# LivGen/LMAT

Hardware: AMD Instinct MI355X
Metric: reads/s (150 bp) vs 64 GB k-mer DB (higher is better)
Workload: dtype u64; 1 GPU; 1104000000 x 150 bp reads/GPU vs 64 GiB k-mer hash (6467472668 20-mers, replicated per GPU), run_rl.sh flags -x 0 -j 30 -l 0 -b 1, calls-only; total_reads=1104000000, reads_per_launch=8000000, read_len=150, db_kmers=6467472668, k=20, parallelism=reads sharded x1, DB replicated, genus_block_permille=100, prune_g=0, list_replicas=1, distinct_lists=792576, reads_called=1058323347, read_pool_batches=32

## Files before the change

### lmat_amd/csrc/kernels.hip

```cpp
#include <hip/hip_runtime.h>
#include <atomic>
#include <type_traits>
#include "kernels.hpp"

#ifndef LMAT_ABLATE
#define LMAT_ABLATE 0
#endif
#define STOP_AT(n, v) do { if (LMAT_ABLATE && A.prm.stop_after == (n)) { if (lane == 0) { emit(250, (v)); } return; } } while (0)
#ifndef LMAT_CLOSURE_FAST
#define LMAT_CLOSURE_FAST 1
#endif
#ifndef LMAT_LDS_SHIFT
#define LMAT_LDS_SHIFT 0
#endif

namespace lmat {

#define WSYNC()                                              \
    do {                                                     \
        __builtin_amdgcn_fence(__ATOMIC_SEQ_CST, "wavefront"); \
        __builtin_amdgcn_wave_barrier();                     \
    } while (0)

template <bool GMEM>
// ... 1011 lines not shown
    float log_avg, stdev1;
    const float sc = k4_wave_stats(lane, nT, cand, my_cnt, xch, log_avg, stdev1);
    const float diff_thresh = stdev1 * Ap->prm.sdiff;
    const float s0 = __uint_as_float(rl(__float_as_uint(sc), (int)sx0));
    const float d = s0 - sc;
    uint64_t close = bal(d <= diff_thresh) & OTH;
    uint8_t match = LMAT_MT_DIRECT;
    uint32_t call_tid = rl(my_id, (int)sx0);
    float call_score = s0;
    if (close) {
        uint64_t good = CH;
        do {
            const uint32_t ivj = rl(fz.z, __builtin_ctzll(close));
            close &= close - 1;
            good &= bal(ti < (ivj & 0xFFFFu)) & bal((ivj >> 16) <= oi);
        } while (close && good);
        if (!good) {
            match = LMAT_MT_LCA_ERROR; call_tid = 0; call_score = 0;
        } else {
            const uint32_t k = wave_max_u32(lane_bit(good) ? (ti << 6) | (uint32_t)lane : 0u);
            match = LMAT_MT_MULTI; call_tid = rl(my_id, (int)(k & 63u));
        }
    }
    k4_wave_closed_record(Ap, lane, out, match, call_tid, call_score, cand, log_avg, stdev1, valid_kmers, len, bin_sel);
    return true;
}
#if LMAT_ABLATE
__device__ uint32_t g_path_why[16];
#define PATH_WHY(i) do { if (lane == 0) atomicAdd(&g_path_why[i], 1u); } while (0)
#else
#define PATH_WHY(i) ((void)0)
#endif
__device__ __forceinline__ bool k4_wave_path(CArgsK4* Ap, int lane, uint32_t nT, uint32_t cand, const u32x4 fz, uint32_t my_cnt,
                                             uint32_t my_id, uint32_t dep, uint32_t fl, uint32_t chain, uint32_t* xch, GAS uint64_t* out,
                                             int valid_kmers, uint32_t len, int bin_sel) {
    const uint32_t nK = (chain >> 8) & 0x7Fu;
    PATH_WHY(0);
    if (nK - 1u >= nT) { PATH_WHY(2); return false; }
    const uint64_t am = below_mask_1_64((int)nT);
    const uint32_t kv = wave_max_u32((uint32_t)lane < nK ? (my_cnt << 6) | (uint32_t)lane : 0u);
    const uint32_t v = kv & 63u, c0 = kv >> 6;
    const uint32_t ti = fz.z & 0xFFFFu, oi = fz.z >> 16;
    const uint32_t riv = rl(fz.z, (int)v);
    const uint32_t rt = riv & 0xFFFFu, ro = riv >> 16;
    const uint64_t CH = bal(ti < rt) & bal(ro <= oi) & am, PATH = CH | (1ull << v), OTH = am & ~PATH;
    if (!CH) { PATH_WHY(3); return false; }
    if (~bal(my_cnt < c0) & OTH) { PATH_WHY(4); return false; }
    if (~bal(my_cnt >= c0) & CH) { PATH_WHY(5); return false; }
    if (~(bal(oi < rt) | bal(ro < ti)) & OTH) { PATH_WHY(6); return false; }
    if (!(bal(dep == 0u) & CH)) { PATH_WHY(7); return false; }
    const uint32_t badfl = (uint32_t)kFlagPlasmid | (Ap->prm.screen_phix ? (uint32_t)kFlagPhiX : 0u);
    if (bal((fl & badfl) != 0)) { PATH_WHY(8); return false; }
    float log_avg, stdev1;
    const float sc = k4_wave_stats(lane, nT, cand, my_cnt, xch, log_avg, stdev1);
    const float diff_thresh = stdev1 * Ap->prm.sdiff;
    const float s0 = __uint_as_float(rl(__float_as_uint(sc), (int)v));
    uint64_t close = bal(s0 - sc <= diff_thresh) & OTH;
    uint8_t match = LMAT_MT_DIRECT;
    uint32_t call_tid = rl(my_id, (int)v);
    float call_score = s0;
    if (close) {
        uint64_t good = CH;
        do {
            const int j = __builtin_ctzll(close);
            close &= close - 1;
            const uint32_t ivj = rl(fz.z, j);
            const float sj = __uint_as_float(rl(__float_as_uint(sc), j));
            const uint64_t anc = bal(ti < (ivj & 0xFFFFu)) & bal((ivj >> 16) <= oi);
            if (bal(sc - sj > diff_thresh) & PATH & ~anc) { PATH_WHY(9); return false; }
            good &= anc;
        } while (close);
        if (!good) {
            match = LMAT_MT_LCA_ERROR; call_tid = 0; call_score = 0;
        } else {
            const uint32_t k = wave_max_u32(lane_bit(good) ? (ti << 6) | (uint32_t)lane : 0u);
            match = LMAT_MT_MULTI; call_tid = rl(my_id, (int)(k & 63u));
            call_score = __uint_as_float(wave_max_u32(lane_bit(PATH) && ti >= (k >> 6) ? __float_as_uint(sc) : 0u));
        }
    }
    PATH_WHY(1);
    k4_wave_closed_record(Ap, lane, out, match, call_tid, call_score, cand, log_avg, stdev1, valid_kmers, len, bin_sel);
    return true;
}
template <int THM, bool PLAIN = false>
__device__ __forceinline__ bool k4_wave(CArgsK4* Ap, int lane, uint32_t nT, uint32_t cand, const u32x4 fz, uint32_t my_cnt,
                                        uint32_t my_id, const unsigned int* hent, uint32_t* xch, GAS uint64_t* out,
                                        int valid_kmers, uint32_t len, int bin_sel, uint32_t chain = 0, uint32_t* took_chain = nullptr) {
    const float hbias = PLAIN ? 0.0f : Ap->prm.hbias, sdiff = Ap->prm.sdiff;
    const int screen_phix = Ap->prm.screen_phix;
    if (!PLAIN && !(Ap->prm.k4_static & 1)) return false;
    const int stop = LMAT_ABLATE ? Ap->prm.stop_after : 0;
    auto placeholder = [&]() {
        if (lane == 0) {
            uint32_t z = 0;
            asm volatile("" : "+v"(z));
            out[0] = (uint64_t)(z + ((uint32_t)LMAT_ST_SILENT | ((uint32_t)LMAT_MT_NOMATCH << 8) | (cand << 16))) | ((uint64_t)(uint32_t)valid_kmers << 32);
            out[1] = (uint64_t)len | ((uint64_t)z << 32);
            out[2] = (uint64_t)z | ((uint64_t)z << 32);
            out[3] = (uint64_t)z | ((uint64_t)z << 32);
            out[4] = (uint64_t)z | ((uint64_t)(uint32_t)bin_sel << 32);
        }
        return true;
    };
    if (stop == 30 || (stop == 34 && nT <= 16)) return placeholder();
    if (cand - 1u > 998u || nT - 1u > 63u) return false;
    const bool act = (uint32_t)lane < nT;
    const uint32_t dep = act ? (fz.w & 0xFFFFu) : 0u, fl = act ? (fz.w >> 16) : 0u;
    if (bal(my_cnt > cand) | bal(dep > 0x7FFFu) | (hbias != 0.0f ? bal((fl & kFlagHuman) != 0) : 0ull)) return false;
    if (LMAT_ABLATE && lane == 0) { G_ADD((GAS uint32_t*)Ap->cursor + kCurChainSeen, 1u); if (chain & 0x10000u) G_ADD((GAS uint32_t*)Ap->cursor + kCurChainLone, 1u); }
    if ((chain & 0x10000u) && (PLAIN || (Ap->prm.k4_static & 4)) &&
        k4_wave_chain(Ap, lane, nT, cand, fz, my_cnt, my_id, dep, fl, chain, xch, out, valid_kmers, len, bin_sel)) {
        if (LMAT_ABLATE && lane == 0) G_ADD((GAS uint32_t*)Ap->cursor + kCurChainTaken, 1u);
        if (took_chain) *took_chain = 1u;
        return true;
    }
    if ((chain & 0x20000u) && (PLAIN || (Ap->prm.k4_static & 8))) {
        if (LMAT_ABLATE && lane == 0) G_ADD((GAS uint32_t*)Ap->cursor + kCurPathSeen, 1u);
        if (k4_wave_path(Ap, lane, nT, cand, fz, my_cnt, my_id, dep, fl, chain, xch, out, valid_kmers, len, bin_sel)) {
            if (LMAT_ABLATE && lane == 0) G_ADD((GAS uint32_t*)Ap->cursor + kCurPathTaken, 1u);
            if (took_chain) *took_chain = 2u;
            return true;
        }
    }
    float* xs = (float*)xch;
    uint32_t* xk = xch + 64;
    uint32_t* xx = xch + 128;
    float* xv = (float*)(xch + 256);
    uint32_t* xp = xch + 320;
    const float fcand = (float)cand;
    const float sc = div_small_ints((float)my_cnt, fcand);
    xs[lane] = sc;
    uint32_t e = act ? (((my_cnt << 15) | dep) << 6) | (uint32_t)lane : 0xFFFFFFFFu;
    if (nT > 16) {
        int lg = 0;
        for (uint32_t t = nT; t > 1; t >>= 1) ++lg;
        uint32_t st0 = 0, st1 = 0, st2 = 0;
        int sp = 0, first = 0, last = (int)nT, depth = 2 * lg;
        bool busy = true;
        while (busy) {
            if (last - first <= 16) {
                if (sp > 0) {
                    --sp;
                    const uint32_t top = sp == 0 ? st0 : (sp == 1 ? st1 : st2);
                    first = (int)(top & 0xFFu); last = (int)((top >> 8) & 0xFFu); depth = (int)(top >> 16);
                } else busy = false;
            } else if (depth == 0) {
                return false;
            } else {
                --depth;
                const int ia = first + 1, ib = first + (last - first) / 2, ic = last - 1;
                const uint32_t ka = rl(e, ia) >> 6, kb = rl(e, ib) >> 6, kc = rl(e, ic) >> 6;
                const bool ab = ka < kb, bc = kb < kc, ac = ka < kc;
                const int pick = ab ? (bc ? ib : (ac ? ic : ia)) : (ac ? ia : (bc ? ic : ib));
                const uint32_t e_first = rl(e, first), e_pick = rl(e, pick);
                e = lane == first ? e_pick : (lane == pick ? e_first : e);
                const uint32_t K = e_pick >> 6;
                const uint64_t inr = below_mask(last) & ~below_mask(first + 1);
                const uint64_t GE = bal((e >> 6) >= K) & inr, LE = bal((e >> 6) <= K) & inr;
                const uint32_t pg = prefix_count(GE), pl = prefix_count(LE);
                const bool le = lane_bit(LE);
                const uint32_t above_le = (uint32_t)popc64(LE) - pl - (le ? 1u : 0u);
                const uint64_t SL = bal(above_le > pg) & GE;
                const uint64_t SR = bal(pg > above_le) & LE;
                int cut;
                if (SL) {
                    const bool swl = lane_bit(SL), swr = lane_bit(SR);
                    if (swl) xx[pg] = e;
                    if (swr) xx[64 + above_le] = e;
                    WSYNC();
                    if (swl) e = xx[64 + pg];
                    if (swr) e = xx[above_le];
                    WSYNC();
                    const int Lm = 63 - __builtin_clzll(SL), Rm = __builtin_ctzll(SR);
                    const uint64_t c = GE & ~below_mask(Lm + 1) & below_mask(Rm);
                    cut = c ? __builtin_ctzll(c) : Rm;
                } else {
                    cut = GE ? __builtin_ctzll(GE) : last;
                }
                if (last - cut > 16) {
                    const uint32_t v = (uint32_t)cut | ((uint32_t)last << 8) | ((uint32_t)depth << 16);
                    if (sp == 0) st0 = v; else if (sp == 1) st1 = v; else st2 = v;
                    ++sp;
                }
                last = cut;
            }
        }
    }
    const uint32_t keyr = act ? ((e & ~63u) | (uint32_t)lane) : 0xFFFFFFFFu;
    xk[lane] = keyr;
    WSYNC();
    float log_sum = 0.0f;
    uint32_t rank = 0;
    for (uint32_t t = 0; t < nT; t += 4) {
        const u32x4 q = *(const u32x4*)((const uint32_t*)xs + t);
        log_sum += __uint_as_float(q.x); log_sum += __uint_as_float(q.y); log_sum += __uint_as_float(q.z); log_sum += __uint_as_float(q.w);
        const u32x4 kq = *(const u32x4*)(xk + t);
        rank += (kq.x < keyr ? 1u : 0u) + (kq.y < keyr ? 1u : 0u) + (kq.z < keyr ? 1u : 0u) + (kq.w < keyr ? 1u : 0u);
    }
    const uint32_t pos_sig_hits = (uint32_t)popc64(bal(my_cnt > 0));
    const uint32_t use_sig_hits = pos_sig_hits > 3 ? pos_sig_hits : nT;
    const float log_avg = div_small_ints(log_sum, (float)use_sig_hits);
    const float dv = log_avg - sc;
    xv[lane] = act && (pos_sig_hits > 3 ? my_cnt > 0 : true) ? dv * dv : 0.0f;
// ... 1676 lines not shown
#pragma unroll
        for (int ch = 0; ch < EC; ++ch) {
            sreg[ch] = 0;
            if ((uint32_t)ch * 64 < nel) {
                const uint32_t e = (uint32_t)ch * 64 + lane;
                if (e < nel) {
                    const uint32_t sl = hent[tid_find(hent, THM, el_ta[e])] >> 16;
                    const bool el = !(dfl[el_d[e]] & kListNegFirst) && ((ES >> sl) & 1ull);
                    sreg[ch] = sl | (el ? 0x100u : 0u);
                    el_ta[e] = (uint16_t)sreg[ch];
                    if (el) atomicMin(&first[sl], e);
                }
            }
        }
        WSYNC();
        STOP_AT(43, nT);
        const uint64_t todo0 = __ballot(first[lane] != 0xFFFFFFFFu);
        const bool one = LMAT_CLOSURE_FAST && todo0 != 0 && (todo0 & (todo0 - 1)) == 0;
        const int sx0 = one ? __builtin_ctzll(todo0) : 0;
        if (one) {
            W = (uint32_t)__builtin_amdgcn_readlane((int)f_plen, sx0);
        } else {
#pragma unroll
            for (int ch = 0; ch < EC; ++ch) {
                if ((uint32_t)ch * 64 < nel) {
                    const uint32_t e = (uint32_t)ch * 64 + lane;
                    const uint32_t sl = sreg[ch] & 0xFFu;
                    const uint32_t plen = lane_of(f_plen, sl);
                    const bool walk = e < nel && first[sl] == e;
                    const uint32_t w = walk ? plen : 0u;
                    const uint32_t incl = wave_scan_incl(w);
                    if (e < nel) el_off[e] = (uint16_t)(W + incl - w);
                    W += (uint32_t)__builtin_amdgcn_readlane((int)incl, 63);
                }
            }
            WSYNC();
        }
        STOP_AT(44, W);
        if (W > 65535u) overflow = true;
        for (uint32_t i0 = 0; i0 < W && !overflow; i0 += 64) {
            const uint32_t i = i0 + lane;
            const bool act = i < W;
            uint32_t a = 0, h = 0;
            uint64_t pe = 0;
            uint32_t sl_i = 0, rel = 0;
            if (one) {
                sl_i = (uint32_t)sx0;
                rel = i;
            } else if (act) {
                uint32_t lo = 0, hi = nel;
                while (lo < hi) {
                    const uint32_t mid = (lo + hi) >> 1;
                    if ((uint32_t)el_off[mid] <= i) lo = mid + 1; else hi = mid;
                }
                const uint32_t e = lo - 1;
                sl_i = (uint32_t)el_ta[e] & 0xFFu;
                rel = i - (uint32_t)el_off[e];
            }
            const uint32_t poff_i = lane_of(f_poff, sl_i);
            uint32_t pf = 0;
            if (act) {
                pe = g_paths8[poff_i + rel];
                pf = ((const GAS uint8_t*)tb.paths_fl)[poff_i + rel];
                a = (uint32_t)(pe & 0xFFFFu);
                h = tid_find_or_claim(hent, THM, a);
                atomicMin(&hent[h], a | ((0x8000u | (uint32_t)lane) << 16));
            }
            WSYNC();
            const uint64_t nm_ = __ballot(i < W) & __ballot((hent[h] >> 16) == (0x8000u | (uint32_t)lane));
            const uint32_t newcnt = popc64(nm_);
            if (nT + newcnt > (uint32_t)T) { overflow = true; break; }
            if (lane_bit(nm_)) {
                const uint32_t s = nT + prefix_count(nm_);
                hent[h] = a | (s << 16);
                reg[s] = (uint16_t)a;
                anc_zw[s] = u32x2{(uint32_t)(pe >> 32), ((uint32_t)(pe >> 16) & 0xFFFFu) | (pf << 16)};
            }
            nT += newcnt;
            WSYNC();
        }
        STOP_AT(45, nT);
        if (!overflow && (uint32_t)lane >= nT_p1 && (uint32_t)lane < nT) { const u32x2 zw = anc_zw[lane]; fz = u32x4{0u, 0u, zw.x, zw.y}; }
        const bool lone = one && !overflow && W > 0 && nT - nT_p1 == W && cand == nuniq;
        if (!overflow) chain = 0x20000u | (nT_p1 << 8);
        if (lone) {
            const uint32_t c0 = cnt[sx0];
            if ((uint32_t)lane >= nT_p1 && (uint32_t)lane < nT) cnt[lane] = (uint16_t)c0;
            chain |= 0x10000u | (uint32_t)sx0;
            WSYNC();
        } else if (!overflow && W > 0) {
            const bool sl_act = (uint32_t)lane < nT;
            uint32_t tin_s = 0xFFFF, tout_s = 0;
            if (sl_act) { tin_s = fz.z & 0xFFFFu; tout_s = fz.z >> 16; }
            uint32_t anc_lo = 0, anc_hi = 0;
            uint64_t todo = todo0;
            while (todo) {
                const int sx = __builtin_ctzll(todo);
                todo &= todo - 1;
                const uint32_t tin_x = (uint32_t)__builtin_amdgcn_readlane((int)tin_s, sx);
                const uint32_t tout_x = (uint32_t)__builtin_amdgcn_readlane((int)tout_s, sx);
                const uint64_t am = __ballot(tin_s < tin_x) & __ballot(tout_x <= tout_s);
                uint32_t m0_keep;
                asm("s_mov_b32 %2, m0\n\ts_mov_b32 m0, %4\n\tv_writelane_b32 %0, %3, m0\n\tv_writelane_b32 %1, %5, m0\n\ts_mov_b32 m0, %2"
                    : "+v"(anc_lo), "+v"(anc_hi), "=&s"(m0_keep) : "s"((uint32_t)am), "s"(sx), "s"((uint32_t)(am >> 32)));
            }
            unsigned int* memw = (unsigned int*)el_t;
            unsigned int* hitw = (unsigned int*)el_off;
            static_assert(2 * E >= 512 && sizeof(*el_t) == 2 && sizeof(*el_off) == 2, "64 mask pairs fit each of the two dead arrays");
            *(u32x2*)(memw + 2 * lane) = u32x2{0u, 0u};
            *(u32x2*)(hitw + 2 * lane) = u32x2{0u, 0u};
            const bool wide_t = nT > 32u;
            WSYNC();
#pragma unroll
            for (int ch = 0; ch < EC; ++ch) {
                if ((uint32_t)ch * 64 < nel) {
                    const uint32_t e = (uint32_t)ch * 64 + lane;
                    const uint32_t se = e < nel ? (uint32_t)el_ta[e] : 0u;
                    const uint32_t sl = se & 0xFFu;
                    const uint32_t alo = lane_of(anc_lo, sl), ahi = wide_t ? lane_of(anc_hi, sl) : 0u;
                    if (e < nel) {
                        const uint32_t d2 = 2u * (uint32_t)el_d[e];
                        __hip_atomic_fetch_or(&memw[d2 + (sl >> 5)], 1u << (sl & 31u), __ATOMIC_RELAXED, __HIP_MEMORY_SCOPE_WORKGROUP);
                        if (se & 0x100u) {
                            __hip_atomic_fetch_or(&hitw[d2], alo, __ATOMIC_RELAXED, __HIP_MEMORY_SCOPE_WORKGROUP);
                            if (wide_t) __hip_atomic_fetch_or(&hitw[d2 + 1], ahi, __ATOMIC_RELAXED, __HIP_MEMORY_SCOPE_WORKGROUP);
                        }
                    }
                }
            }
            WSYNC();
            {
                const u32x2 me = *(const u32x2*)(memw + 2 * lane), hi_ = *(const u32x2*)(hitw + 2 * lane);
                *(u32x2*)(hitw + 2 * lane) = u32x2{hi_.x & ~me.x, hi_.y & ~me.y};
            }
            WSYNC();
            const unsigned int* aw = hitw + (lane >> 5);
            const uint32_t sh = (uint32_t)lane & 31u;
            uint32_t add = 0;
            auto mad_lo = [](uint32_t bit, uint32_t mm, uint32_t acc) -> uint32_t { uint32_t r; asm("v_mad_u32_u16 %0, %1, %2, %3" : "=v"(r) : "v"(bit), "v"(mm), "v"(acc)); return r; };
            auto mad_hi = [](uint32_t bit, uint32_t mm, uint32_t acc) -> uint32_t { uint32_t r; asm("v_mad_u32_u16 %0, %1, %2, %3 op_sel:[0,1,0,0]" : "=v"(r) : "v"(bit), "v"(mm), "v"(acc)); return r; };
            static_assert(L::D == 64 && (L::OFF_R2 + 4 * L::D) % 8 == 0, "the multiplicities are read eight bytes at a time, up to set 63");
            for (uint32_t d = 0; d < ndist; d += 4) {
                const unsigned int* pw = aw + 2 * d;
                const uint32_t w0 = pw[0], w1 = pw[2], w2 = pw[4], w3 = pw[6];
                const u32x2 mm = *(const u32x2*)(dmult + d);
                add = mad_lo(__builtin_amdgcn_ubfe(w0, sh, 1u), mm.x, add);
                add = mad_hi(__builtin_amdgcn_ubfe(w1, sh, 1u), mm.x, add);
                add = mad_lo(__builtin_amdgcn_ubfe(w2, sh, 1u), mm.y, add);
                add = mad_hi(__builtin_amdgcn_ubfe(w3, sh, 1u), mm.y, add);
            }
            if (sl_act && add) cnt[lane] = (uint16_t)(cnt[lane] + add);
            WSYNC();
        }
    }
    if (overflow) {
        if (lane == 0) {
            emit(255, 0);
            if (A.ovf_list) ((GAS uint32_t*)A.ovf_list)[G_ADD(&g_cursor[A.ovf_slot], 1u)] = (uint32_t)r;
            else G_OR(g_err, (uint32_t)kErrTidOverflow);
        }
        return;
    }
    STOP_AT(6, nT);
    if (!PLAIN && A.rand_max) {
        const uint32_t gcb = ((const GAS uint8_t*)A.rand_gc)[r - A.result_base];
        GAS uint32_t* rmax = (GAS uint32_t*)A.rand_max;
        GAS uint32_t* rcnt = (GAS uint32_t*)A.rand_cnt;
// ... 664 lines not shown
    if (!n) return;
    probe_stats_kernel<<<dim3((unsigned)((n + 255) / 256)), dim3(256), 0, stream>>>(tb, kmers, n, out);
}

void launch_gather_bench(const uint64_t* slots, uint32_t nbuckets, uint64_t n_probes, uint64_t seed,
                         unsigned long long* sink, hipStream_t stream, int bytes_per_probe) {
    const int grid = 256 * 16;
    if (bytes_per_probe == 128) {
        const uint64_t per_wave = (n_probes / grid + 71) / 72 * 72;
        gather_bench_kernel<8><<<dim3(grid), dim3(64), 0, stream>>>(slots, nbuckets, per_wave, seed, sink);
    } else {
        const uint64_t per_wave = (n_probes / grid + 143) / 144 * 144;
        gather_bench_kernel<4><<<dim3(grid), dim3(64), 0, stream>>>(slots, nbuckets, per_wave, seed, sink);
    }
}

template <int TT>
static void launch_k4_lds(const ClassifyArgs& a, uint64_t max_reads, hipStream_t stream) {
    using K = K4Lds<TT>;
    static PerDeviceOnce attr_once;
    attr_once([] { hipFuncSetAttribute((const void*)k4_lds_kernel<TT>, hipFuncAttributeMaxDynamicSharedMemorySize, K::BYTES); });
    const uint64_t per_cu = 160 * 1024 / K::BYTES;
    uint64_t g = (max_reads + K::LANES - 1) / K::LANES;
    if (g > 256 * per_cu) g = 256 * per_cu;
    static const int gcap = getenv("LMAT_K4_SMALL_GRID") ? atoi(getenv("LMAT_K4_SMALL_GRID")) : 0;
    if (TT == kK4SmallT && gcap > 0 && g > (uint64_t)gcap) g = gcap;
    if (g < 1) g = 1;
    k4_lds_kernel<TT><<<dim3((unsigned)g), dim3(64), K::BYTES, stream>>>(a);
}
void launch_k4_begin(const ClassifyArgs& a, hipStream_t stream, hipStream_t stream2, hipStream_t stream3, hipStream_t small_stream,
                     hipEvent_t forked) {
    uint64_t blocks = (a.count + 4095) / 4096;
    if (blocks > 256 * 8) blocks = 256 * 8;
    if (blocks < 1) blocks = 1;
    k4_compact_kernel<<<dim3((unsigned)blocks), dim3(256), 0, stream>>>(a);
    hipEventRecord(forked, stream);
    hipStreamWaitEvent(stream2, forked, 0);
    ClassifyArgs b = a;
    b.k4_slot = kCurK4Large;
    const uint64_t waves = (a.count + 63) / 64;
    uint64_t g2 = waves < 256 * 32 ? waves : 256 * 32;
    if (g2 < 1) g2 = 1;
    static const int g2cap = getenv("LMAT_K4_MID_GRID") ? atoi(getenv("LMAT_K4_MID_GRID")) : 0;
    if (g2cap > 0 && g2 > (uint64_t)g2cap) g2 = g2cap;
    else if (small_stream == stream3 && g2 > 1024) g2 = 1024;
    static const int mode = getenv("LMAT_K4_MODE") ? atoi(getenv("LMAT_K4_MODE")) : 0;
    if (a.nm.active) {
        k4_kernel<true, kK4T, 64><<<dim3((unsigned)g2), dim3(64), 0, stream2>>>(b);
    } else if (mode == 1) {
        launch_k4_lds<kK4MidT>(a, a.count, stream2);
    } else {
        b.k4_slot = kCurK4Mid;
        k4_kernel<false, kK4MidT, 64><<<dim3((unsigned)g2), dim3(64), 0, stream2>>>(b);
    }
    hipStreamWaitEvent(stream3, forked, 0);
    if (!a.nm.active && a.prm.k4_row) {
        uint64_t gr = (a.count + 3) / 4;
        if (gr > 256 * 64) gr = 256 * 64;
        if (gr < 1) gr = 1;
        k4_row_kernel<<<dim3((unsigned)gr), dim3(64), 0, stream3>>>(a);
    }
    if (!a.nm.active) launch_k4_lds<kK4T>(a, a.count / 8 + 64, stream3);
    if (small_stream != stream && small_stream != stream3) hipStreamWaitEvent(small_stream, forked, 0);
    launch_k4_lds<kK4SmallT>(a, a.count, small_stream);
}
void launch_k4_end(const ClassifyArgs& a, hipStream_t join_stream, hipStream_t stream2, hipStream_t stream3, hipStream_t small_stream,
                   hipEvent_t joined2, hipEvent_t joined3, hipEvent_t joined_small, hipEvent_t done) {
    if (stream2 != join_stream) { hipEventRecord(joined2, stream2); hipStreamWaitEvent(join_stream, joined2, 0); }
    if (stream3 != join_stream) { hipEventRecord(joined3, stream3); hipStreamWaitEvent(join_stream, joined3, 0); }
    if (small_stream != join_stream && small_stream != stream3 && small_stream != stream2) {
        hipEventRecord(joined_small, small_stream);
        hipStreamWaitEvent(join_stream, joined_small, 0);
    }
    ClassifyArgs b = a;
    b.k4_slot = kCurK4Bail;
    if (a.nm.active) k4_kernel<true, kK4T, 64><<<dim3(64), dim3(64), 0, join_stream>>>(b);
    else k4_kernel<false, kK4T, 64><<<dim3(64), dim3(64), 0, join_stream>>>(b);
    hipEventRecord(done, join_stream);
}

static int k4_static_of(const ClassifyArgs& a) {
    const int stop = a.prm.stop_after;
    const bool base = !a.nm.active && a.tb.depth_consistent && !(a.cands && !a.prm.prn_all);
    const bool wave = base && (stop == 0 || (stop >= 30 && stop <= 34));
    const bool rows = base && a.prm.k4_row && stop == 0;
    const bool closed = wave && stop == 0 && !a.cands;
    return (wave ? 1 : 0) | (rows ? 2 : 0) | (closed && (a.prm.k4_chain & 1) ? 4 : 0) | (closed && (a.prm.k4_chain & 2) ? 8 : 0);
}
static bool plain_launch(const ClassifyArgs& a, int k4_static) {
    static const bool on = !LMAT_ABLATE && (!getenv("LMAT_PLAIN") || atoi(getenv("LMAT_PLAIN")) != 0);
    return on && a.tb.k == 20 && a.tb.cpt.nb && a.tb.cpt.m == 17 && a.tb.cpt.lowbits == 2 && !a.tb.wide && !a.nm.active && !a.rand_max &&
           !a.gene_mode && !a.prm.permissive && a.prm.stop_after == 0 && k4_static == 13 && !a.cands && a.prm.hbias == 0.0f &&
           a.p_min == 0 && a.p_max == 0xFFFFFFFFu && !a.index && !a.count_ptr && a.tail_lpr == 4;
}
static bool uniform_launch(const ClassifyArgs& a) {
    static const bool on = !getenv("LMAT_UNIFORM") || atoi(getenv("LMAT_UNIFORM")) != 0;
    return on && a.uniform;
}
static std::atomic<unsigned long long> g_variant_launches[64][3];
void classify_variant_launches(int device, uint64_t out[2]) {
    out[0] = out[1] = 0;
    if (device < 0 || device >= 64) return;
    out[0] = g_variant_launches[device][0].load();
    out[1] = g_variant_launches[device][1].load();
}
uint64_t classify_uniform_launches(int device) { return device < 0 || device >= 64 ? 0 : g_variant_launches[device][2].load(); }
template <int U, int T, int E, bool INK4, bool PERM, bool CPT, bool WIDE = false, bool PLAIN = false, bool UNI = false>
static void launch_classify_t(const ClassifyArgs& a_in, hipStream_t stream) {
    using L = WL<U, T, E, INK4, CPT, WIDE>;
    ClassifyArgs a = a_in;
    a.prm.k4_static = k4_static_of(a);
    constexpr bool kPlainClass = U == 160 && T == 64 && E == kFastE && !INK4 && !PERM && CPT && !WIDE;
    if constexpr (kPlainClass && !PLAIN && !LMAT_ABLATE) {
        if (plain_launch(a, a.prm.k4_static)) {
            if (uniform_launch(a)) launch_classify_t<U, T, E, INK4, PERM, CPT, WIDE, true, true>(a_in, stream);
            else launch_classify_t<U, T, E, INK4, PERM, CPT, WIDE, true>(a_in, stream);
            return;
        }
    }
    if constexpr (kPlainClass) {
        int dev = 0;
        if (hipGetDevice(&dev) == hipSuccess && dev >= 0 && dev < 64) {
            g_variant_launches[dev][PLAIN ? 1 : 0]++;
            if (UNI) g_variant_launches[dev][2]++;
        }
    }
    if (U > 2048) {
        int grid = kGmemGrid;
        if (!a.count_ptr && (uint64_t)grid > a.count) grid = (int)(a.count ? a.count : 1);
        classify_kernel<U, T, E, INK4, PERM, CPT, WIDE><<<dim3(grid), dim3(64), CPT ? L::XL_BYTES : 0, stream>>>(a);
        return;
    }
    static const int lds_pad = getenv("LMAT_LDS_PAD") ? atoi(getenv("LMAT_LDS_PAD")) : 0;
    const int lds_bytes = L::BYTES + lds_pad;
    static PerDeviceOnce attr_once;
    attr_once([lds_bytes] { hipFuncSetAttribute((const void*)classify_kernel<U, T, E, INK4, PERM, CPT, WIDE, PLAIN, UNI>, hipFuncAttributeMaxDynamicSharedMemorySize, lds_bytes); });
    const int per_cu = 160 * 1024 / lds_bytes;
    static const int gmult = getenv("LMAT_GRID_MULT") ? atoi(getenv("LMAT_GRID_MULT")) : 32;
    int grid = 256 * (per_cu < 1 ? 1 : (per_cu > 32 ? 32 : per_cu)) * (gmult > 0 ? gmult : 32);
    if (!a.count_ptr && (uint64_t)grid > a.count) grid = (int)a.count;
    if (a.count_ptr && INK4 && grid > 256 * (per_cu < 2 ? 2 : per_cu)) grid = 256 * (per_cu < 2 ? 2 : per_cu);
    if (grid < 1) grid = 1;
    classify_kernel<U, T, E, INK4, PERM, CPT, WIDE, PLAIN, UNI><<<dim3(grid), dim3(64), lds_bytes, stream>>>(a);
}

void launch_k4_debug(const ClassifyArgs& a, const uint32_t* idx, const float* scores, const uint64_t* off, const float* stdevs, uint64_t n,
                     hipStream_t stream) {
    if (!n) return;
    k4_debug_kernel<<<dim3((unsigned)((n + 63) / 64)), dim3(64), 0, stream>>>(a, idx, scores, off, stdevs, n);
}

void launch_k4_debug_counts(const ClassifyArgs& a, const uint32_t* idx, const uint32_t* cnts, const uint64_t* off, const uint32_t* cands, uint64_t n,
                            bool on_the_wave, hipStream_t stream, const uint32_t* shape, uint8_t* took) {
    if (!n) return;
    if (on_the_wave) {
        const uint64_t g = n < 256 * 32 ? n : 256 * 32;
        ClassifyArgs b = a;
        b.prm.k4_static = k4_static_of(b);
        k4_wave_debug_kernel<<<dim3((unsigned)g), dim3(64), 0, stream>>>(b, idx, cnts, off, cands, n, shape, took);
    } else k4_debug_counts_kernel<<<dim3((unsigned)((n + 63) / 64)), dim3(64), 0, stream>>>(a, idx, cnts, off, cands, n);
}

#if LMAT_ABLATE
}
extern "C" int lmat_ablate_path_why(uint32_t* out16, int reset) {
    if (hipDeviceSynchronize() != hipSuccess) return -1;
    if (out16 && hipMemcpyFromSymbol(out16, HIP_SYMBOL(lmat::g_path_why), 64) != hipSuccess) return -1;
    if (reset) { const uint32_t z[16] = {0}; if (hipMemcpyToSymbol(HIP_SYMBOL(lmat::g_path_why), z, 64) != hipSuccess) return -1; }
    return 0;
}
namespace lmat {
#endif

void launch_tail(const ClassifyArgs& a, hipStream_t stream) {
    if (!a.tail_lpr || !a.count || a.count_ptr) return;
    const uint64_t lanes = a.count * a.tail_lpr;
    const dim3 grid((unsigned)((lanes + 255) / 256));
    if (a.tail_lpr == 4) tail_kernel<4><<<grid, dim3(256), 0, stream>>>(a);
    else if (a.tail_lpr == 8) tail_kernel<8><<<grid, dim3(256), 0, stream>>>(a);
    else tail_kernel<16><<<grid, dim3(256), 0, stream>>>(a);
}

int classify_max_read_len() { return kGmemU + 19; }
size_t classify_gmem_scratch_bytes() { return (size_t)kGmemGrid * WL<kGmemU, 4096, 16384, true, false, true>::BYTES; }

#define LC(U, T, E, K)                                                                                                   \
    (a.tb.cpt.nb ? (a.prm.permissive ? launch_classify_t<U, T, E, K, true, true>(a, stream) : launch_classify_t<U, T, E, K, false, true>(a, stream)) \
                 : (a.prm.permissive ? launch_classify_t<U, T, E, K, true, false>(a, stream) : launch_classify_t<U, T, E, K, false, false>(a, stream)))
#define LCW(U, T, E) (a.prm.permissive ? launch_classify_t<U, T, E, true, true, true, true>(a, stream) : launch_classify_t<U, T, E, true, false, true, true>(a, stream))
bool launch_classify(const ClassifyArgs& a, uint32_t max_read_len, int tcap_class, hipStream_t stream) {
    const int k = a.tb.k;
    const uint32_t P = max_read_len >= (uint32_t)k ? max_read_len - k + 1 : 0;
    if (a.tb.wide) {
        if (!a.tb.cpt.nb) return false;
        if (tcap_class == 4) { if (P > 512) return false; LCW(512, 128, 512); }
        else if (tcap_class == 5) { if (P <= 512) LCW(512, 512, 2048); else if (P <= 2048) LCW(2048, 512, 2048); else return false; }
        else if (P <= (uint32_t)kGmemU && a.gscratch) LCW(kGmemU, 4096, 16384);
        else return false;
        return true;
    }
    if (tcap_class == 2) {
        if (P <= 160) LC(160, 64, 512, false); else LC(512, 64, 512, false);
    } else if (tcap_class == 3) {
        if (P > 512) return false;
        LC(512, 256, 1024, true);
    } else if (P <= 160 && tcap_class == 0) {
        LC(160, 64, kFastE, false);
    } else if (P <= 256) {
        if (tcap_class == 0) LC(256, 64, kFastE, false); else LC(256, 1024, 4096, true);
    } else if (P <= 320 && tcap_class == 0) {
        LC(320, 64, kFastE, false);
    } else if (P <= 512) {
        if (tcap_class == 0) LC(512, 64, kFastE, false); else LC(512, 1024, 4096, true);
    } else if (P <= 2048) {
        LC(2048, 1024, 4096, true);
    } else if (P <= (uint32_t)kGmemU && a.gscratch) {
        LC(kGmemU, 4096, 16384, true);
    } else {
        return false;
    }
    return true;
}

uint32_t synth_strain_base_host(const SynthGeo& g, uint32_t species, uint32_t strain_global, uint64_t pos) {
    return synth_strain_base(g, species, strain_global, pos);
}
void synth_window_host(const SynthGeo& g, int k, uint32_t species, uint64_t pos, uint64_t* kmer, uint32_t* first_strain, uint32_t* mask, bool* inblk,
                       int* cons_level) {
    const int clv = synth_cons_window(g, pos, k);
    if (cons_level) *cons_level = clv;
    if (clv >= 0) {
        const uint32_t sp0 = species - species % g.csz[clv];
        uint64_t anc = 0;
        for (int j = 0; j < k; ++j) anc = (anc << 2) | synth_anc_base(g, sp0, pos + j);
        *kmer = canon_from_fwd(anc, k);
        *first_strain = sp0 * g.S;
        *mask = 0;
        *inblk = false;
        return;
    }
    const bool blk = pos + k <= g.blk;
    const uint32_t sp = blk ? species - species % g.spg : species;
    uint64_t anc = 0;
    for (int j = 0; j < k; ++j) anc = (anc << 2) | synth_anc_base(g, sp, pos + j);
    const uint32_t ns = blk ? g.spg * g.S : g.S;
    uint32_t m = 0;
// ... 45 lines not shown
```

### lmat_amd/csrc/lmat_api.cpp

```cpp
#include <hip/hip_runtime.h>
#include <algorithm>
#include <cmath>
#include <cstdio>
#include <cstring>
#include <chrono>
#include <string>
#include <thread>
#include <atomic>
#include <fcntl.h>
#include <unistd.h>
#include "kernels.hpp"
#include "outfmt.hpp"

using namespace lmat;

#define HIPCHK(ctx, call)                                                                          \
    do {                                                                                           \
        hipError_t e__ = (call);                                                                   \
        if (e__ != hipSuccess)                                                                     \
            return set_err(ctx, LMAT_E_DEVICE, std::string(#call) + ": " + hipGetErrorString(e__)); \
    } while (0)

template <class T>
static int dev_upload(lmat_ctx* c, T** dst, const std::vector<T>& src) {
    if (*dst) { hipFree(*dst); *dst = nullptr; }
    size_t bytes = std::max<size_t>(src.size(), 1) * sizeof(T);
    HIPCHK(c, hipMalloc((void**)dst, bytes));
    if (!src.empty()) HIPCHK(c, hipMemcpy(*dst, src.data(), src.size() * sizeof(T), hipMemcpyHostToDevice));
    return LMAT_OK;
}

namespace lmat {
int upload_taxonomy(lmat_ctx* c) {
    HostTaxonomy& T = c->tax;
    int rc;
    if ((rc = dev_upload(c, &c->dev.tid32, T.tid32))) return rc;
    if ((rc = dev_upload(c, &c->dev.fdepth, T.fdepth))) return rc;
    if ((rc = dev_upload(c, &c->dev.flags, T.flags))) return rc;
    if ((rc = dev_upload(c, &c->dev.path_off, T.path_off))) return rc;
    if ((rc = dev_upload(c, &c->dev.path_len, T.path_len))) return rc;
    if ((rc = dev_upload(c, &c->dev.conv, T.conv))) return rc;
    c->dev.wide = T.wide ? 1u : 0u;
    if (T.wide) {
        if ((rc = dev_upload(c, &c->dev.species_of32, T.species_of))) return rc;
        if ((rc = dev_upload(c, &c->dev.paths32, T.paths))) return rc;
        if ((rc = dev_upload(c, &c->dev.tin32, T.tin))) return rc;
        if ((rc = dev_upload(c, &c->dev.tout32, T.tout))) return rc;
    } else {
        auto narrow = [](const std::vector<uint32_t>& v) { return std::vector<uint16_t>(v.begin(), v.end()); };
        if ((rc = dev_upload(c, &c->dev.species_of, narrow(T.species_of)))) return rc;
        if ((rc = dev_upload(c, &c->dev.paths, narrow(T.paths)))) return rc;
        if ((rc = dev_upload(c, &c->dev.tin, narrow(T.tin)))) return rc;
        if ((rc = dev_upload(c, &c->dev.tout, narrow(T.tout)))) return rc;
        std::vector<uint64_t> p8(T.paths.size());
        std::vector<uint8_t> pfl(T.paths.size());
        for (size_t i = 0; i < T.paths.size(); ++i) {
            const uint32_t a = T.paths[i];
            p8[i] = (uint64_t)a | ((uint64_t)T.fdepth[a] << 16) | ((uint64_t)T.tin[a] << 32) | ((uint64_t)T.tout[a] << 48);
            pfl[i] = (uint8_t)T.flags[a];
        }
        if ((rc = dev_upload(c, &c->dev.paths_fl, pfl))) return rc;
        std::vector<uint32_t> f16((size_t)(T.n + 1) * 4);
        for (uint32_t i = 0; i <= T.n; ++i) {
            f16[4 * i + 0] = T.path_off[i];
            f16[4 * i + 1] = (uint32_t)T.path_len[i] | ((uint32_t)T.species_of[i] << 16);
            f16[4 * i + 2] = (uint32_t)T.tin[i] | ((uint32_t)T.tout[i] << 16);
            f16[4 * i + 3] = (uint32_t)T.fdepth[i] | ((uint32_t)T.flags[i] << 16);
        }
        if ((rc = dev_upload(c, &c->dev.paths8, p8))) return rc;
        if ((rc = dev_upload(c, &c->dev.facts16, f16))) return rc;
    }
    c->dev.n_ids = T.n + 1;
    c->dev.depth_consistent = 1;
    for (uint32_t i = 1; i <= T.n; ++i)
        if (T.path_len[i] && T.fdepth[i] <= T.fdepth[T.paths[T.path_off[i]]]) { c->dev.depth_consistent = 0; break; }
    if (c->d_counts) { hipFree(c->d_counts); c->d_counts = nullptr; }
    c->counts_bytes = (uint64_t)c->dev.n_ids * 16 + 24;
    HIPCHK(c, hipMalloc(&c->d_counts, c->counts_bytes));
    HIPCHK(c, hipMemset(c->d_counts, 0, c->counts_bytes));
    return LMAT_OK;
}
}

static KernelParams kparams(const lmat_params& p) {
    KernelParams k;
    k.sdiff = p.sdiff; k.hbias = p.hbias; k.min_score = p.min_score;
    k.min_kmer = p.min_kmer; k.min_fnd_kmer = p.min_fnd_kmer; k.prn_all = p.prn_all; k.screen_phix = p.screen_phix;
    k.permissive = 0;
    const char* sa = getenv("LMAT_STOP_AFTER");
    k.stop_after = sa ? atoi(sa) : 0;
    if (const char* w = getenv("LMAT_K4_WAVE")) if (!k.stop_after && atoi(w) == 0) k.stop_after = 20;
    k.k4_row = getenv("LMAT_K4_ROW") && atoi(getenv("LMAT_K4_ROW")) != 0;
    k.k4_chain = !(getenv("LMAT_K4_CHAIN") && atoi(getenv("LMAT_K4_CHAIN")) == 0) ? 1 : 0;
    if (!(getenv("LMAT_K4_PATH") && atoi(getenv("LMAT_K4_PATH")) == 0)) k.k4_chain |= 2;
    k.k4_static = 0;
    return k;
}

extern "C" {

static void sb_free(lmat_ctx* c);
static int sb_begin(lmat_ctx* c, uint64_t n_kmers, uint64_t table_bytes, int k);
static int sb_push(lmat_ctx* c, Ingest& B);

int lmat_device_count(void) {
    int n = 0;
    return hipGetDeviceCount(&n) == hipSuccess ? n : 0;
}

int lmat_ctx_create(int device, const lmat_params* params, lmat_ctx** out) {
    if (!out) return LMAT_E_ARG;
    *out = nullptr;
    int ndev = 0;
    if (hipGetDeviceCount(&ndev) != hipSuccess || ndev <= 0 || device < 0 || device >= ndev) return LMAT_E_DEVICE;
    if (hipSetDevice(device) != hipSuccess) return LMAT_E_DEVICE;
    lmat_ctx* c = new lmat_ctx();
    c->device = device;
    lmat_params def = {1.0f, 3.0f, 0.0f, 35, 1, 0, 1};
    c->params = params ? *params : def;
    if (hipStreamCreate(&c->stream) != hipSuccess) { delete c; return LMAT_E_DEVICE; }
    if (c->sets[0].cursor.ensure(kCursorBytes) != hipSuccess || c->sets[1].cursor.ensure(kCursorBytes) != hipSuccess ||
        hipMalloc((void**)&c->d_err, 64) != hipSuccess) { delete c; return LMAT_E_DEVICE; }
    for (auto& s : c->sets) hipMemset(s.cursor.p, 0, kCursorBytes);
    hipMemset(c->d_err, 0, 64);
    *out = c;
    return LMAT_OK;
}

void lmat_ctx_destroy(lmat_ctx* c) {
    if (!c) return;
    hipSetDevice(c->device);
    hipDeviceSynchronize();
    for (auto& e : c->pending_events) { hipEventDestroy(e.first); hipEventDestroy(e.second); }
    for (auto& e : c->pending_events2) { hipEventDestroy(e.first); hipEventDestroy(e.second); }
    void* ptrs[] = {c->dev.slots, c->dev.ovf_slots, c->dev.arena, c->dev.tid32, c->dev.fdepth, c->dev.flags, c->dev.species_of,
                    c->dev.path_off, c->dev.path_len, c->dev.paths, c->dev.paths8, c->dev.paths_fl, c->dev.facts16, c->dev.conv, c->dev.tin, c->dev.tout, c->dev.paths32, c->dev.tin32, c->dev.tout32, c->dev.species_of32,
                    c->d_counts, c->d_synth_strain_idx, c->d_rand_max, c->d_rand_cnt, c->d_err};
    for (void* p : ptrs)
        if (p) hipFree(p);
    sb_free(c);
    free_null_models(c);
    comm_free(c);
    if (c->ev_fork) hipEventDestroy(c->ev_fork);
    if (c->ev_join) hipEventDestroy(c->ev_join);
    if (c->ev_join3) hipEventDestroy(c->ev_join3);
    if (c->ev_join_small) hipEventDestroy(c->ev_join_small);
    if (c->stream3) hipStreamDestroy(c->stream3);
    if (c->stream2) hipStreamDestroy(c->stream2);
    if (c->stream) hipStreamDestroy(c->stream);
    delete c->ingest;
    delete c;
}

const char* lmat_last_error(const lmat_ctx* c) { return c ? c->err.c_str() : "null context"; }

int lmat_set_params(lmat_ctx* c, const lmat_params* p) {
    if (!c || !p) return LMAT_E_ARG;
    c->params = *p;
    return LMAT_OK;
}

int lmat_taxonomy_load_files(lmat_ctx* c, const char* tree_fn, const char* depth_fn, const char* rank_fn,
                             const char* idmap_fn, const char* plasmid_fn) {
    if (!c) return LMAT_E_ARG;
    hipSetDevice(c->device);
    return load_taxonomy_files(c, tree_fn, depth_fn, rank_fn, idmap_fn, plasmid_fn);
}

int lmat_ingest_create(int k, const char* idmap_fn, lmat_ingest** out) {
    if (!out || k < 1 || k > 20) return LMAT_E_ARG;
    lmat_ingest* g = new lmat_ingest();
    g->ing.k = k;
    if (idmap_fn && *idmap_fn && !g->ing.load_idmap(idmap_fn)) { delete g; *out = nullptr; return LMAT_E_IO; }
    *out = g;
    return LMAT_OK;
}
int lmat_ingest_idmap_from_tree(lmat_ingest* g, const char* tree_fn) {
// ... 1619 lines not shown
    int rc = debug_tables(c, tids, nullptr, n ? off[n] : 0, idx);
    if (rc || !n) return rc;
    hipSetDevice(c->device);
    const uint64_t total = off[n];
    DevBuf d_idx, d_sc, d_sd, d_off, d_res;
    if ((rc = debug_put(c, d_idx, idx.data(), total * 4)) || (rc = debug_put(c, d_sc, scores, total * 4)) ||
        (rc = debug_put(c, d_sd, stdev, n * 4)) || (rc = debug_put(c, d_off, off, (n + 1) * 8))) return rc;
    HIPCHK(c, d_res.ensure(n * sizeof(lmat_read_result)));
    ClassifyArgs a;
    a.tb = c->dev;
    a.prm = kparams(c->params);
    a.prm.stop_after = 0;
    a.results = d_res.as<lmat_read_result>();
    a.nm = NullModelDev();
    launch_k4_debug(a, d_idx.as<uint32_t>(), d_sc.as<float>(), d_off.as<uint64_t>(), d_sd.as<float>(), n, c->stream);
    if ((rc = debug_fetch(c, d_res, n, results))) return rc;
    for (uint64_t i = 0; i < n; ++i)
        if (results[i].status == 255) return set_err(c, LMAT_E_CAPACITY, "a candidate table outside 1..64 entries, or a lineage beyond the scratch");
    return LMAT_OK;
}

static int debug_decide_counts(lmat_ctx* c, const uint32_t* tids, const uint32_t* counts, const uint64_t* off, const uint32_t* cand, uint64_t n,
                               int on_the_wave, const std::vector<uint32_t>* shape, int with_cands, lmat_read_result* results, uint8_t* took) {
    std::vector<uint32_t> idx;
    int rc = debug_tables(c, tids, counts, n ? off[n] : 0, idx);
    if (rc || !n) return rc;
    hipSetDevice(c->device);
    const uint64_t total = off[n];
    DevBuf d_idx, d_cn, d_cd, d_off, d_res, d_tally, d_shape, d_took, d_cands;
    HIPCHK(c, d_tally.ensure(c->counts_bytes));
    HIPCHK(c, hipMemsetAsync(d_tally.p, 0, c->counts_bytes, c->stream));
    if ((rc = debug_put(c, d_idx, idx.data(), total * 4)) || (rc = debug_put(c, d_cn, counts, total * 4)) ||
        (rc = debug_put(c, d_cd, cand, n * 4)) || (rc = debug_put(c, d_off, off, (n + 1) * 8))) return rc;
    HIPCHK(c, d_res.ensure(n * sizeof(lmat_read_result)));
    const lmat_ctx::BatchSet& s = c->set();
    HIPCHK(c, hipMemsetAsync(s.cursor.p, 0, kCursorWords * 4, c->stream));
    ClassifyArgs a;
    a.tb = c->dev;
    a.prm = kparams(c->params);
    a.prm.stop_after = 0;
    a.results = d_res.as<lmat_read_result>();
    a.cands = nullptr;
    a.cand_cap = 0;
    a.cursor = s.word(0);
    a.err = c->d_err;
    a.counts = d_tally.p;
    auto it = c->tax.index_of.find(32630);
    a.phix_call_idx = it == c->tax.index_of.end() ? 0 : it->second;
    a.nm = NullModelDev();
    if (shape && (rc = debug_put(c, d_shape, shape->data(), n * 4))) return rc;
    if (took) HIPCHK(c, d_took.ensure(n));
    if (with_cands) {
        HIPCHK(c, d_cands.ensure(total * sizeof(lmat_cand)));
        a.cands = d_cands.as<lmat_cand>();
        a.cand_cap = total;
        a.prm.prn_all = 1;
    }
    launch_k4_debug_counts(a, d_idx.as<uint32_t>(), d_cn.as<uint32_t>(), d_off.as<uint64_t>(), d_cd.as<uint32_t>(), n, on_the_wave != 0, c->stream,
                           shape ? d_shape.as<uint32_t>() : nullptr, took ? d_took.as<uint8_t>() : nullptr);
    if (took) HIPCHK(c, hipMemcpyAsync(took, d_took.p, n, hipMemcpyDeviceToHost, c->stream));
    return debug_fetch(c, d_res, n, results);
}
int lmat_debug_decide_counts(lmat_ctx* c, const uint32_t* tids, const uint32_t* counts, const uint64_t* off, const uint32_t* cand, uint64_t n,
                             int on_the_wave, lmat_read_result* results) {
    if (!c || !tids || !counts || !off || !cand || !results) return LMAT_E_ARG;
    return debug_decide_counts(c, tids, counts, off, cand, n, on_the_wave, nullptr, 0, results, nullptr);
}
int lmat_debug_decide_chain(lmat_ctx* c, const uint32_t* tids, const uint32_t* counts, const uint64_t* off, const uint32_t* cand,
                            const uint32_t* kept, const uint32_t* eligible, uint64_t n, int with_cands, lmat_read_result* results, uint8_t* took) {
    if (!c || !tids || !counts || !off || !cand || !kept || !eligible || !results || !took) return LMAT_E_ARG;
    std::vector<uint32_t> shape(n);
    for (uint64_t i = 0; i < n; ++i) {
        if (kept[i] > 64u || (kept[i] && eligible[i] >= kept[i])) return set_err(c, LMAT_E_ARG, "kept slots above 64, or an eligible slot that is not among them");
        shape[i] = kept[i] ? (0x10000u | (kept[i] << 8) | eligible[i]) : 0u;
    }
    return debug_decide_counts(c, tids, counts, off, cand, n, 1, &shape, with_cands, results, took);
}
int lmat_debug_decide_shape(lmat_ctx* c, const uint32_t* tids, const uint32_t* counts, const uint64_t* off, const uint32_t* cand,
                            const uint32_t* shape, uint64_t n, int with_cands, lmat_read_result* results, uint8_t* took) {
    if (!c || !tids || !counts || !off || !cand || !shape || !results || !took) return LMAT_E_ARG;
    std::vector<uint32_t> sh(shape, shape + n);
    for (uint64_t i = 0; i < n; ++i) {
        const uint32_t kept = (sh[i] >> 8) & 0xFFu, el = sh[i] & 0xFFu;
        if ((sh[i] & ~0x3FFFFu) || kept > 64u || ((sh[i] & 0x10000u) && el >= kept) || (!(sh[i] & 0x10000u) && el) || (!(sh[i] & 0x30000u) && sh[i]))
            return set_err(c, LMAT_E_ARG, "a shape word with kept slots above 64, an eligible slot that is not among them, or bits without their flag");
    }
    return debug_decide_counts(c, tids, counts, off, cand, n, 1, &sh, with_cands, results, took);
}

int lmat_debug_last_counters(lmat_ctx* c, uint32_t* out16) {
    if (!c || !out16) return LMAT_E_ARG;
    hipSetDevice(c->device);
    HIPCHK(c, hipMemcpy(out16, c->set().cursor.p, kCursorWords * 4, hipMemcpyDeviceToHost));
    return LMAT_OK;
}

int lmat_debug_variant_launches(lmat_ctx* c, uint64_t* out2) {
    if (!c || !out2) return LMAT_E_ARG;
    classify_variant_launches(c->device, out2);
    return LMAT_OK;
}
int lmat_debug_uniform_launches(lmat_ctx* c, uint64_t* out) {
    if (!c || !out) return LMAT_E_ARG;
    *out = classify_uniform_launches(c->device);
    return LMAT_OK;
}

int lmat_last_timing(const lmat_ctx* c, float* classify_ms, float* decide_ms, uint64_t* launches) {
    if (!c) return LMAT_E_ARG;
    if (classify_ms) *classify_ms = c->last_classify_ms;
    if (decide_ms) *decide_ms = c->last_decide_ms;
    if (launches) *launches = c->last_launches;
    return LMAT_OK;
}

int lmat_results_fetch(lmat_ctx* c, uint64_t first, uint64_t count, lmat_read_result* results) {
    if (!c || !results || (first + count) * sizeof(lmat_read_result) > c->set().results.bytes) return LMAT_E_ARG;
    hipSetDevice(c->device);
    HIPCHK(c, hipMemcpy(results, c->set().results.as<lmat_read_result>() + first, count * sizeof(lmat_read_result), hipMemcpyDeviceToHost));
    return LMAT_OK;
}

int lmat_counts_reset(lmat_ctx* c) {
    if (!c || !c->d_counts) return LMAT_E_ARG;
    hipSetDevice(c->device);
    HIPCHK(c, hipMemsetAsync(c->d_counts, 0, c->counts_bytes, c->stream));
    HIPCHK(c, hipStreamSynchronize(c->stream));
    return LMAT_OK;
}
int lmat_counts_layout(const lmat_ctx* c, uint32_t* n_ids, uint64_t* bytes) {
    if (!c) return LMAT_E_ARG;
    if (n_ids) *n_ids = c->dev.n_ids;
    if (bytes) *bytes = c->counts_bytes;
    return LMAT_OK;
}
void* lmat_counts_device_ptr(lmat_ctx* c) { return c ? c->d_counts : nullptr; }

int lmat_counts_get(lmat_ctx* c, uint32_t* tid32, uint64_t* count, double* score, uint32_t cap, uint32_t* n_nonzero,
                    uint64_t nomatch3[3]) {
    if (!c || !c->d_counts) return LMAT_E_ARG;
    hipSetDevice(c->device);
    HIPCHK(c, hipStreamSynchronize(c->stream));
    std::vector<unsigned char> buf(c->counts_bytes);
    HIPCHK(c, hipMemcpy(buf.data(), c->d_counts, c->counts_bytes, hipMemcpyDeviceToHost));
    const uint32_t n = c->dev.n_ids;
    const uint64_t* cn = (const uint64_t*)buf.data();
    const double* sc = (const double*)(cn + n);
    const uint64_t* nm = (const uint64_t*)(sc + n);
    uint32_t k = 0;
    for (uint32_t i = 0; i < n; ++i)
        if (cn[i]) {
            if (k < cap) {
                if (tid32) tid32[k] = c->tax.tid32[i];
                if (count) count[k] = cn[i];
                if (score) score[k] = sc[i];
            }
            ++k;
        }
    if (n_nonzero) *n_nonzero = k;
    if (nomatch3) { nomatch3[0] = nm[0]; nomatch3[1] = nm[1]; nomatch3[2] = nm[2]; }
    return LMAT_OK;
}

int lmat_gather_bench(lmat_ctx* c, uint64_t n_probes, uint64_t seed, float* ms, uint64_t* bytes) {
    if (!c || !c->db_ready) return set_err(c, LMAT_E_ARG, "database not ready");
    hipSetDevice(c->device);
    unsigned long long* sink = nullptr;
// ... 391 lines not shown
```

Baseline: 430.4 million reads/s.

## Add closed-form tie resolver for multi-top-count reads in wave decide

Adds a k4_wave_tie fast path that resolves reads where several kept taxa tie on the top count at equal depth. It classifies ancestors into common and private sets using interval containment and emits the LCA call directly, avoiding the general wave sort/merge path. It is enabled by a new shape flag bit and on by default via k4_chain bit 4, and the plain-launch static mask is updated to match. It adds extra ballot work and register pressure to the shared kernel, and the long chain of bail-out conditions must reproduce the reference LCA semantics exactly.

```diff
diff --git a/lmat_amd/csrc/kernels.hip b/lmat_amd/csrc/kernels.hip
--- a/lmat_amd/csrc/kernels.hip
+++ b/lmat_amd/csrc/kernels.hip
@@ -1117,6 +1117,87 @@
     k4_wave_closed_record(Ap, lane, out, match, call_tid, call_score, cand, log_avg, stdev1, valid_kmers, len, bin_sel);
     return true;
 }
+#if LMAT_ABLATE
+__device__ uint32_t g_tie_why[32];
+#define TIE_WHY(i) do { if (lane == 0) atomicAdd(&g_tie_why[i], 1u); } while (0)
+#else
+#define TIE_WHY(i) ((void)0)
+#endif
+__device__ __forceinline__ bool k4_wave_tie(CArgsK4* Ap, int lane, uint32_t nT, uint32_t cand, const u32x4 fz, uint32_t my_cnt,
+                                            uint32_t my_id, uint32_t dep, uint32_t fl, uint32_t chain, uint32_t* xch, GAS uint64_t* out,
+                                            int valid_kmers, uint32_t len, int bin_sel) {
+    const uint32_t nK = (chain >> 8) & 0x7Fu;
+    TIE_WHY(0);
+    if (nK < 2u || nK >= nT) { TIE_WHY(2); return false; }
+    const uint64_t am = below_mask_1_64((int)nT), KEPT = below_mask_1_64((int)nK);
+    const uint32_t ti = fz.z & 0xFFFFu, oi = fz.z >> 16;
+    const uint32_t kv = wave_max_u32((uint32_t)lane < nK ? (my_cnt << 22) | (ti << 6) | (uint32_t)lane : 0u);
+    const uint32_t c0 = kv >> 22, tmax = (kv >> 6) & 0xFFFFu, v = kv & 63u;
+    const uint64_t EQ = bal(my_cnt == c0), GT = bal(my_cnt > c0) & am, TOP = EQ & KEPT;
+    if (!(TOP & (TOP - 1)) || c0 == 0u) { TIE_WHY(3); return false; }
+    const uint32_t D = rl(dep, (int)v);
+    if (~bal(dep == D) & TOP) { TIE_WHY(4); return false; }
+    const uint32_t tmin = 0xFFFFu - wave_max_u32(lane_bit(TOP) ? 0xFFFFu - ti : 0u);
+    const uint64_t COMMON = bal(ti < tmin) & bal(tmax <= oi) & am;
+    uint64_t PRIVATE = 0;
+    uint32_t nabove = (uint32_t)popc64(COMMON);
+    for (uint64_t t = bal(dep < D) & am & ~COMMON; t; t &= t - 1) {
+        const int j = __builtin_ctzll(t);
+        const uint32_t ivj = rl(fz.z, j);
+        const uint64_t under = bal((ivj & 0xFFFFu) < ti) & bal(ti <= (ivj >> 16)) & TOP;
+        if (under) PRIVATE |= 1ull << j;
+        nabove += lane_bit(under) ? 1u : 0u;
+    }
+    if (LMAT_ABLATE) TIE_WHY(GT & (COMMON | PRIVATE) ? 16 : 17);
+    if (bal(nabove != (fz.y & 0xFFFFu)) & TOP) { TIE_WHY(5); return false; }
+    if (!COMMON) { TIE_WHY(6); return false; }
+    const uint64_t REST = am & ~COMMON & ~PRIVATE & ~TOP;
+    if (GT & ~COMMON) { TIE_WHY(7); return false; }
+    if (~EQ & PRIVATE) { TIE_WHY(8); return false; }
+    if (EQ & REST) { TIE_WHY(9); return false; }
+    if (~(GT | EQ) & COMMON) { TIE_WHY(10); return false; }
+    if (GT) {
+        const uint32_t key = (my_cnt << 16) | ti;
+        for (uint64_t t = GT; t; t &= t - 1) {
+            const uint32_t kj = rl(key, __builtin_ctzll(t));
+            if (bal(ti < (kj & 0xFFFFu)) & bal(my_cnt < (kj >> 16)) & COMMON) { TIE_WHY(10); return false; }
+        }
+    }
+    if (COMMON & KEPT) { TIE_WHY(11); return false; }
+    if (!(bal(dep == 0u) & COMMON)) { TIE_WHY(12); return false; }
+    const uint32_t badfl = (uint32_t)kFlagPlasmid | (Ap->prm.screen_phix ? (uint32_t)kFlagPhiX : 0u);
+    if (bal((fl & badfl) != 0)) { TIE_WHY(13); return false; }
+    for (uint64_t t = bal(dep > D) & REST; t; t &= t - 1) {
+        const uint32_t ivj = rl(fz.z, __builtin_ctzll(t));
+        if (bal(ti < (ivj & 0xFFFFu)) & bal((ivj >> 16) <= oi) & TOP) { TIE_WHY(14); return false; }
+    }
+    float log_avg, stdev1;
+    const float sc = k4_wave_stats(lane, nT, cand, my_cnt, xch, log_avg, stdev1);
+    const float diff_thresh = stdev1 * Ap->prm.sdiff;
+    if (!(diff_thresh >= 0.0f)) { TIE_WHY(15); return false; }
+    const float s0 = __uint_as_float(rl(__float_as_uint(sc), (int)v));
+    const uint64_t LIN = GT ? GT : COMMON;
+    uint64_t close = bal(s0 - sc <= diff_thresh) & REST, good = LIN;
+    while (close) {
+        const int j = __builtin_ctzll(close);
+        close &= close - 1;
+        const uint32_t ivj = rl(fz.z, j);
+        const float sj = __uint_as_float(rl(__float_as_uint(sc), j));
+        const uint64_t anc = bal(ti < (ivj & 0xFFFFu)) & bal((ivj >> 16) <= oi);
+        if (bal(sc - sj > diff_thresh) & LIN & ~anc) { TIE_WHY(15); return false; }
+        good &= anc;
+    }
+    uint8_t match = LMAT_MT_LCA_ERROR;
+    uint32_t call_tid = 0;
+    float call_score = 0;
+    if (good) {
+        const uint32_t k = wave_max_u32(lane_bit(good) ? (ti << 6) | (uint32_t)lane : 0u) & 63u;
+        match = LMAT_MT_MULTI; call_tid = rl(my_id, (int)k); call_score = __uint_as_float(rl(__float_as_uint(sc), (int)k));
+    }
+    TIE_WHY(1);
+    k4_wave_closed_record(Ap, lane, out, match, call_tid, call_score, cand, log_avg, stdev1, valid_kmers, len, bin_sel);
+    return true;
+}
 template <int THM, bool PLAIN = false>
 __device__ __forceinline__ bool k4_wave(CArgsK4* Ap, int lane, uint32_t nT, uint32_t cand, const u32x4 fz, uint32_t my_cnt,
                                         uint32_t my_id, const unsigned int* hent, uint32_t* xch, GAS uint64_t* out,
@@ -1154,6 +1235,17 @@
         if (k4_wave_path(Ap, lane, nT, cand, fz, my_cnt, my_id, dep, fl, chain, xch, out, valid_kmers, len, bin_sel)) {
             if (LMAT_ABLATE && lane == 0) G_ADD((GAS uint32_t*)Ap->cursor + kCurPathTaken, 1u);
             if (took_chain) *took_chain = 2u;
+            return true;
+        }
+    }
+    if ((chain & 0x40000u) && (PLAIN || (Ap->prm.k4_static & 16))) {
+        if (LMAT_ABLATE && stop == 35) {
+            const uint32_t nK = (chain >> 8) & 0x7Fu;
+            const uint32_t kv = wave_max_u32((uint32_t)lane < nK ? (my_cnt << 6) | (uint32_t)lane : 0u);
+            const uint64_t TOP = bal(my_cnt == (kv >> 6)) & below_mask_1_64((int)(nK ? nK : 1u));
+            if (nK >= 2u && (TOP & (TOP - 1)) && !(~bal(dep == rl(dep, (int)(kv & 63u))) & TOP)) return placeholder();
+        } else if (k4_wave_tie(Ap, lane, nT, cand, fz, my_cnt, my_id, dep, fl, chain, xch, out, valid_kmers, len, bin_sel)) {
+            if (took_chain) *took_chain = 3u;
             return true;
         }
     }
@@ -2996,7 +3088,7 @@
         STOP_AT(45, nT);
         if (!overflow && (uint32_t)lane >= nT_p1 && (uint32_t)lane < nT) { const u32x2 zw = anc_zw[lane]; fz = u32x4{0u, 0u, zw.x, zw.y}; }
         const bool lone = one && !overflow && W > 0 && nT - nT_p1 == W && cand == nuniq;
-        if (!overflow) chain = 0x20000u | (nT_p1 << 8);
+        if (!overflow) chain = 0x60000u | (nT_p1 << 8);
         if (lone) {
             const uint32_t c0 = cnt[sx0];
             if ((uint32_t)lane >= nT_p1 && (uint32_t)lane < nT) cnt[lane] = (uint16_t)c0;
@@ -3827,15 +3919,16 @@
 static int k4_static_of(const ClassifyArgs& a) {
     const int stop = a.prm.stop_after;
     const bool base = !a.nm.active && a.tb.depth_consistent && !(a.cands && !a.prm.prn_all);
-    const bool wave = base && (stop == 0 || (stop >= 30 && stop <= 34));
+    const bool wave = base && (stop == 0 || (stop >= 30 && stop <= 35));
     const bool rows = base && a.prm.k4_row && stop == 0;
-    const bool closed = wave && stop == 0 && !a.cands;
-    return (wave ? 1 : 0) | (rows ? 2 : 0) | (closed && (a.prm.k4_chain & 1) ? 4 : 0) | (closed && (a.prm.k4_chain & 2) ? 8 : 0);
+    const bool closed = wave && (stop == 0 || stop == 35) && !a.cands;
+    return (wave ? 1 : 0) | (rows ? 2 : 0) | (closed && (a.prm.k4_chain & 1) ? 4 : 0) | (closed && (a.prm.k4_chain & 2) ? 8 : 0) |
+           (closed && (a.prm.k4_chain & 4) ? 16 : 0);
 }
 static bool plain_launch(const ClassifyArgs& a, int k4_static) {
     static const bool on = !LMAT_ABLATE && (!getenv("LMAT_PLAIN") || atoi(getenv("LMAT_PLAIN")) != 0);
     return on && a.tb.k == 20 && a.tb.cpt.nb && a.tb.cpt.m == 17 && a.tb.cpt.lowbits == 2 && !a.tb.wide && !a.nm.active && !a.rand_max &&
-           !a.gene_mode && !a.prm.permissive && a.prm.stop_after == 0 && k4_static == 13 && !a.cands && a.prm.hbias == 0.0f &&
+           !a.gene_mode && !a.prm.permissive && a.prm.stop_after == 0 && k4_static == 29 && !a.cands && a.prm.hbias == 0.0f &&
            a.p_min == 0 && a.p_max == 0xFFFFFFFFu && !a.index && !a.count_ptr && a.tail_lpr == 4;
 }
 static bool uniform_launch(const ClassifyArgs& a) {
@@ -3907,6 +4000,12 @@
 }
 
 #if LMAT_ABLATE
+}
+extern "C" int lmat_ablate_tie_why(uint32_t* out32, int reset) {
+    if (hipDeviceSynchronize() != hipSuccess) return -1;
+    if (out32 && hipMemcpyFromSymbol(out32, HIP_SYMBOL(lmat::g_tie_why), 128) != hipSuccess) return -1;
+    if (reset) { const uint32_t z[32] = {0}; if (hipMemcpyToSymbol(HIP_SYMBOL(lmat::g_tie_why), z, 128) != hipSuccess) return -1; }
+    return 0;
 }
 extern "C" int lmat_ablate_path_why(uint32_t* out16, int reset) {
     if (hipDeviceSynchronize() != hipSuccess) return -1;
diff --git a/lmat_amd/csrc/lmat_api.cpp b/lmat_amd/csrc/lmat_api.cpp
--- a/lmat_amd/csrc/lmat_api.cpp
+++ b/lmat_amd/csrc/lmat_api.cpp
@@ -93,6 +93,7 @@
     k.k4_row = getenv("LMAT_K4_ROW") && atoi(getenv("LMAT_K4_ROW")) != 0;
     k.k4_chain = !(getenv("LMAT_K4_CHAIN") && atoi(getenv("LMAT_K4_CHAIN")) == 0) ? 1 : 0;
     if (!(getenv("LMAT_K4_PATH") && atoi(getenv("LMAT_K4_PATH")) == 0)) k.k4_chain |= 2;
+    if (!(getenv("LMAT_K4_TIE") && atoi(getenv("LMAT_K4_TIE")) == 0)) k.k4_chain |= 4;
     k.k4_static = 0;
     return k;
 }
@@ -1878,7 +1879,8 @@
     std::vector<uint32_t> sh(shape, shape + n);
     for (uint64_t i = 0; i < n; ++i) {
         const uint32_t kept = (sh[i] >> 8) & 0xFFu, el = sh[i] & 0xFFu;
-        if ((sh[i] & ~0x3FFFFu) || kept > 64u || ((sh[i] & 0x10000u) && el >= kept) || (!(sh[i] & 0x10000u) && el) || (!(sh[i] & 0x30000u) && sh[i]))
+        if ((sh[i] & ~0x7FFFFu) || kept > 64u || ((sh[i] & 0x10000u) && el >= kept) || (!(sh[i] & 0x10000u) && el) || (!(sh[i] & 0x30000u) && sh[i]) ||
+            ((sh[i] & 0x40000u) && !(sh[i] & 0x20000u)))
             return set_err(c, LMAT_E_ARG, "a shape word with kept slots above 64, an eligible slot that is not among them, or bits without their flag");
     }
     return debug_decide_counts(c, tids, counts, off, cand, n, 1, &sh, with_cands, results, took);
```

New measurement: 435.6 million reads/s, median of 6. 1.2% higher.
